# fu5ha/rayn

Hardware: AMD Instinct MI355X
Metric: Mpath-samples/sec (higher is better)
Workload: dtype f32; 1 GPU; 1920x1080, 1024 spp, 8 bounces, MandelBox SDF + homogeneous volume [BASELINE configs[2]]; fma_policy=unfused (reference default build), parallelism=tiles round-robin over 1 GPU(s), build_variant=product, resolve_kernel=k_resolve_blk<128, 8>

## Files before the change

rayn_amd/csrc/kernels.hip:

```cpp
#include <hip/hip_runtime.h>

#include <stdlib.h>

#include <algorithm>

#include "device_core.h"
#include "kernels.h"

#if defined(__HIP_DEVICE_COMPILE__) && !defined(__gfx950__)
#error "kernels.hip is written for gfx950 (MI355X): k_resolve_blk<512, 8> / k_resolve_huge use 64 KB / 130 KB of the CU's 160 KB LDS"
#endif

namespace RAYN_KNS {

RD uint32_t lane_id() { return threadIdx.x & 63u; }
RD uint32_t mbcnt(uint64_t mask) {
    return __builtin_amdgcn_mbcnt_hi((uint32_t)(mask >> 32), __builtin_amdgcn_mbcnt_lo((uint32_t)mask, 0u));
}

__global__ void __launch_bounds__(256) k_pack_tables(Tables tab, float4* __restrict__ out, uint32_t spp, uint32_t depths, uint32_t n1, uint32_t n2) {
    const uint32_t r = blockIdx.x * blockDim.x + threadIdx.x;
    if (r >= spp * depths) return;
    const uint32_t depth = r / spp, s = r % spp;
    float* dst = (float*)(out + (size_t)r * tab.rec_stride);
    for (uint32_t k = 0; k < 8; k++) dst[k] = k < n1 ? tab.s1d[s + spp * (1 + k + depth * n1)] : 0.0f;
    for (uint32_t c = 0; c < n2; c++) dst[8 + c] = tab.s2d[(c & 1) + s * 2 + spp * 2 * (2 + (c >> 1) + depth * (n2 / 2))];
}

__global__ void __launch_bounds__(256) k_batch_setup(const DTile* __restrict__ tiles, uint32_t* __restrict__ pgrp_tile,
                                                      uint32_t* __restrict__ tgb, uint32_t* __restrict__ tgc) {
    const uint32_t k = blockIdx.x;
    const DTile t = tiles[k];
    const uint32_t g0 = t.pool_base >> 6, groups = (t.n_paths + 63u) >> 6;
    if (threadIdx.x == 0) { tgb[k] = g0; tgc[k] = groups; }
    for (uint32_t g = threadIdx.x; g < groups; g += 256) pgrp_tile[g0 + g] = k;
}

__global__ void __launch_bounds__(256) k_raygen(const DScene* __restrict__ scp, Tables tab, const float* __restrict__ scramble,
                                                 const DTile* __restrict__ tiles, const uint32_t* __restrict__ pgrp_tile,
                                                 Pool pool, uint32_t* __restrict__ q, uint32_t n_pool, DCtl* __restrict__ ctl) {
    const uint32_t P = blockIdx.x * blockDim.x + threadIdx.x;
    if (P >= n_pool) return;
    if (P == 0) { ctl->q_groups = n_pool >> 6; ctl->q_valid = n_pool; ctl->head_extend = 0; }
    const DScene& sc = *scp;
    const DTile tile = tiles[pgrp_tile[P >> 6]];
    const uint32_t p = P - tile.pool_base;
    pool.term_info[P] = (uint8_t)TERM_NONE;
    pool.aov[P] = make_float4(0.0f, 0.0f, 0.0f, __uint_as_float(OBJ_NONE));
    if (p >= tile.n_paths) { q[P] = INVALID; return; }
    const uint32_t spp = sc.spp;
    const uint32_t s = p % spp, lpix = p / spp;
    const uint32_t lx = lpix / tile.eh, ly = lpix % tile.eh;
    const uint32_t x = tile.x0 + lx, y = tile.y0 + ly;
    const uint32_t pix = x + y * sc.width;
    const float scr = scramble[pix];
    float u0 = sample_2d(tab, spp, 0, s, scr, 0), u1 = sample_2d(tab, spp, 1, s, scr, 0);
    float fx = fis_sample(tab.fis, u0), fy = fis_sample(tab.fis, u1);
    float scx = ((float)x + 0.5f) + fx, scy = ((float)y + 0.5f) + fy;
    float uvx = sc.ndc_x * scx, uvy = sc.ndc_y * scy;
    float time = sc.time_start + sc.time_range * sample_1d(tab, spp, s, scr, 0);
    float l0 = sample_2d(tab, spp, 0, s, scr, 1), l1 = sample_2d(tab, spp, 1, s, scr, 1);
    const float t0 = sc.cam.animated ? sc.time_start + sc.time_range * sample_1d(tab, spp, s & ~3u, scr, 0) : time;
    f3 o, d;
    camera_ray(sc.cam, uvx, uvy, l0, l1, t0, &o, &d);
    pool.geo0[P] = make_float4(o.x, o.y, o.z, d.x);
    pool.geo1[P] = make_float4(d.y, d.z, 0.0f, __uint_as_float(OBJ_NONE | (s << 8)));
    pool.col0[P] = make_float4(0.0f, 0.0f, 0.0f, 1.0f);
    pool.col1[P] = make_float4(1.0f, 1.0f, __uint_as_float(pix), time);
    q[P] = P;
}

RD float packet_time(const DScene& sc, const uint32_t* __restrict__ q, const Pool& pool, uint32_t ent) {
    if (!sc.anim_spheres) return 0.0f;
    const uint32_t P0 = q[ent & ~3u];
    return P0 == INVALID ? dm_nanf() : pool.col1[P0].w;
}

constexpr uint32_t CHUNK = 256;
constexpr uint32_t ENDGAME_ENTRIES = 256 * 32 * 64;

template <bool COUNT>
__global__ void __launch_bounds__(256) k_extend(const DScene* __restrict__ scp, uint32_t depth, const uint32_t* __restrict__ q,
                                                 DCtl* __restrict__ ctl, Pool pool, uint8_t* __restrict__ ent_obj,
                                                 uint32_t REFILL_MIN, unsigned long long* __restrict__ evals_out) {
    const DScene& sc = *scp;
    const uint32_t n_entries = ctl->q_groups << 6;
    uint32_t* const head = &ctl->head_extend;
    const uint32_t lane = lane_id();
    const Thr th = make_thr(sc, depth);
    const uint32_t nh = sc.n_hitables;
    const float c0 = 0.00005f * sc.detail_scale, c1 = 0.05f * sc.detail_scale;
    uint32_t cur = 0, end = 0;
    bool exhausted = false;
    bool has = false, first = false, nan = false;
    uint32_t ent = 0, P = 0, k = 0, id = OBJ_NONE, m = 0, sbits = 0;
    EvalCtr evals;
    f3 o = f3{0, 0, 0}, d = f3{0, 0, 0};
    float closest = 0.0f, t = 0.0f, t0 = 0.0f;
    auto advance = [&]() {
        while (k < nh) {
            const DHitable& hh = sc.h[k];
            if (hh.kind != RAYN_HITABLE_SPHERE) { first = true; return; }
            float ts = sphere_hit(hh, o, d, closest, t0);
            if (ts < closest) { closest = ts; id = k; }
            k++;
        }
        *(float2*)(&pool.geo1[P].z) = make_float2(closest, __uint_as_float((sbits & ~0xFFu) | id));
        ent_obj[ent] = (uint8_t)id;
        has = false;
    };
    bool marching = false;
    for (;;) {
        const uint64_t parked = __ballot(!marching);
        if (parked != 0 && ((uint32_t)__popcll(parked) >= REFILL_MIN || exhausted)) {
            if (has && !marching) { advance(); marching = has; }
            for (;;) {
                const uint64_t need = __ballot(!has);
                if (need == 0) break;
                if (cur == end) {
                    if (exhausted) break;
                    uint32_t base = 0;
                    if (lane == 0) base = atomicAdd(head, CHUNK);
                    base = __builtin_amdgcn_readfirstlane(base);
                    if (base >= n_entries) { exhausted = true; break; }
                    cur = base;
                    end = min(base + CHUNK, n_entries);
                }
                const uint32_t rank = mbcnt(need), avail = end - cur;
                if (!has && rank < avail) {
                    ent = cur + rank;
                    P = q[ent];
                    if (P == INVALID) ent_obj[ent] = (uint8_t)OBJ_NONE;
                    else {
                        const float4 g0 = pool.geo0[P], g1 = pool.geo1[P];
                        o = f3{g0.x, g0.y, g0.z};
                        d = f3{g0.w, g1.x, g1.y};
                        sbits = __float_as_uint(g1.w);
                        t0 = packet_time(sc, q, pool, ent);
                        closest = sc.t_max; id = OBJ_NONE; k = 0; has = true;
                        advance();
                        marching = has;
                    }
                }
                cur += min((uint32_t)__popcll(need), avail);
            }
        }
        const uint64_t act = __ballot(marching);
        if (act == 0) {
            if (__ballot(has) == 0 && exhausted) break;
            continue;
        }
        const uint32_t ku = (uint32_t)__builtin_amdgcn_readlane((int)k, (int)__builtin_ctzll(act));
        const DHitable& h = sc.h[ku];
        if (marching && k == ku) {
            const f3 ol = o - sphere_center(h, t0);
            const f3 p = first ? ol : muladd3(d, t, ol);
            const float dist = sdf_dist<COUNT>(h, p, evals, sdf_scale(h, t0));
            bool done;
            if (first) { t = dist; nan = dist != dist; first = false; m = 0; done = sc.max_marches == 0; }
            else {
                const bool hit = __builtin_fabsf(dist) < fmaxs(c0, c1 * thr_at(th, t));
                const bool gt = t > closest;
                done = hit || nan || gt;
                if (!done) { t = t + dist; m++; done = m == sc.max_marches; }
            }
            if (done) {
                if (t < closest) { closest = t; id = k; }
                k++;
                marching = false;
            }
        }
    }
    if (COUNT && evals.n) { atomicAdd(evals_out, (unsigned long long)evals.n); atomicAdd(evals_out + 4, (unsigned long long)evals.it); }
}

template <bool COUNT, int SDFK>
__global__ void __launch_bounds__(256) k_extend1(const DScene* __restrict__ scp, uint32_t depth, uint32_t ks, const uint32_t* __restrict__ q,
                                                  DCtl* __restrict__ ctl, Pool pool, uint8_t* __restrict__ ent_obj,
                                                  uint32_t PREFETCH_MIN, unsigned long long* __restrict__ evals_out) {
    const DScene& sc = *scp;
    const uint32_t n_entries = ctl->q_groups << 6;
    uint32_t* const head = &ctl->head_extend;
    const uint32_t lane = lane_id();
    const Thr th = make_thr(sc, depth);
    const uint32_t nh = sc.n_hitables, max_marches = sc.max_marches;
    const DHitable h = sc.h[ks];
    const float c0 = 0.00005f * sc.detail_scale, c1 = 0.05f * sc.detail_scale;
    uint32_t cur = 0, end = 0;
    bool exhausted = false, endgame = false;
    bool c_has = false, first = false, nan = false;
    uint32_t c_P = 0, c_ent = 0, c_ids = 0, m = 0;
    EvalCtr evals;
    f3 o = f3{0, 0, 0}, d = f3{0, 0, 0};
    f3 pt = f3{0, 0, 0};
    float c_pre = 0.0f, c_post = 0.0f, t = 0.0f;
    float c_scale = h.scale, n_scale = h.scale;
    bool n_has = false;
    uint32_t n_P = 0, n_ent = 0, n_ids = 0;
    f3 n_o = f3{0, 0, 0}, n_d = f3{0, 0, 0};
    float n_pre = 0.0f, n_post = 0.0f;
    for (;;) {
        const uint64_t lack = __ballot(!n_has);
        const uint64_t idle = __ballot(!c_has && !n_has);
        if (!exhausted && (endgame ? idle != 0 : ((uint32_t)__popcll(lack) >= PREFETCH_MIN || (uint32_t)__popcll(idle) >= 4u))) {
            for (;;) {
                const uint64_t need = endgame ? __ballot(!n_has && !c_has) : __ballot(!n_has);
                if (need == 0) break;
                if (cur == end) {
                    uint32_t base = 0;
                    if (lane == 0) base = atomicAdd(head, CHUNK);
                    base = __builtin_amdgcn_readfirstlane(base);
                    if (base >= n_entries) { exhausted = true; break; }
                    cur = base;
                    end = min(base + CHUNK, n_entries);
                    endgame = n_entries - base < ENDGAME_ENTRIES;
                }
                const uint32_t rank = mbcnt(need), avail = end - cur;
                if ((need >> lane) & 1ull) if (rank < avail) {
                    n_ent = cur + rank;
                    n_P = q[n_ent];
                    if (n_P == INVALID) ent_obj[n_ent] = (uint8_t)OBJ_NONE;
                    else {
                        const float4 g0 = pool.geo0[n_P];
                        const float2 g1 = *(const float2*)(&pool.geo1[n_P].x);
                        n_o = f3{g0.x, g0.y, g0.z};
                        n_d = f3{g0.w, g1.x, g1.y};
                        const float t0 = packet_time(sc, q, pool, n_ent);
                        float closest = sc.t_max;
                        uint32_t id = OBJ_NONE;
                        for (uint32_t k = 0; k < ks; k++) {
                            float ts = sphere_hit(sc.h[k], n_o, n_d, closest, t0);
                            if (ts < closest) { closest = ts; id = k; }
                        }
                        n_pre = closest;
                        uint32_t idp = OBJ_NONE;
                        for (uint32_t k = ks + 1; k < nh; k++) {
                            float ts = sphere_hit(sc.h[k], n_o, n_d, closest, t0);
                            if (ts < closest) { closest = ts; idp = k; }
                        }
                        n_post = closest;
                        n_ids = id | (idp << 8);
                        n_o = n_o - sphere_center(h, t0);
                        n_scale = sdf_scale(h, t0);
                        n_has = true;
                    }
                }
                cur += min((uint32_t)__popcll(need), avail);
            }
        }
        if (!c_has && n_has) {
            c_has = true; n_has = false;
            o = n_o; d = n_d; c_pre = n_pre; c_post = n_post; c_ids = n_ids; c_P = n_P; c_ent = n_ent; c_scale = n_scale;
            first = true;
#ifndef RAYN_MARCH_POINT_SELECT
            pt = n_o;
#endif
        }
        if (__ballot(c_has) == 0) {
            if (exhausted) break;
            continue;
        }
        if (c_has) {
#ifdef RAYN_MARCH_POINT_SELECT
            const f3 p = first ? o : muladd3(d, t, o);
#else
            const f3 p = pt;
#endif
            const float dist = sdf_dist<COUNT, SDFK>(h, p, evals, c_scale);
            bool done;
            if (first) { t = dist; nan = dist != dist; first = false; m = 0; done = max_marches == 0; }
            else {
                const bool hit = __builtin_fabsf(dist) < fmaxs(c0, c1 * thr_at(th, t));
                const bool gt = t > c_pre;
                done = hit || nan || gt;
                if (!done) { t = t + dist; m++; done = m == max_marches; }
            }
            if (done) {
                float closest = c_pre;
                uint32_t id = c_ids & 0xFFu;
                if (t < closest) { closest = t; id = ks; }
                const uint32_t idp = c_ids >> 8;
                if (idp != OBJ_NONE && c_post < closest) { closest = c_post; id = idp; }
                pool.geo1[c_P].z = closest;
                ((uint8_t*)&pool.geo1[c_P].w)[0] = (uint8_t)id;
                ent_obj[c_ent] = (uint8_t)id;
                c_has = false;
            }
#ifndef RAYN_MARCH_POINT_SELECT
            else pt = muladd3(d, t, o);
#endif
        }
    }
    if (COUNT && evals.n) { atomicAdd(evals_out, (unsigned long long)evals.n); atomicAdd(evals_out + 4, (unsigned long long)evals.it); }
}

constexpr uint32_t QUEUE_UNROLL = 8;

RD uint32_t quad_total(uint32_t n) {
    n += (uint32_t)__builtin_amdgcn_update_dpp(0, (int)n, 0xB1, 0xF, 0xF, true);
    n += (uint32_t)__builtin_amdgcn_update_dpp(0, (int)n, 0x4E, 0xF, 0xF, true);
    return n;
}
RD uint32_t count_eq4(uint32_t v, uint32_t pat) {
    const uint32_t x = v ^ pat;
    return (uint32_t)__popc(~(((x & 0x7F7F7F7Fu) + 0x7F7F7F7Fu) | x | 0x7F7F7F7Fu));
}
__global__ void __launch_bounds__(256) k_group_hist(uint32_t nclass, const uint8_t* __restrict__ ent_obj, const DCtl* __restrict__ ctl,
                                                     uint8_t* __restrict__ grp_cnt) {
    const uint32_t n_q = ctl->q_groups << 2;
    const uint4* __restrict__ obj16 = (const uint4*)ent_obj;
    const uint32_t stride = gridDim.x * blockDim.x;
    constexpr uint32_t HIST_UNROLL = 2;
    for (uint32_t i0 = blockIdx.x * blockDim.x + threadIdx.x; i0 < n_q; i0 += stride * HIST_UNROLL) {
        uint4 v[HIST_UNROLL];
#pragma unroll
        for (uint32_t u = 0; u < HIST_UNROLL; u++) { const uint32_t i = i0 + u * stride; v[u] = i < n_q ? obj16[i] : make_uint4(~0u, ~0u, ~0u, ~0u); }
#pragma unroll
        for (uint32_t u = 0; u < HIST_UNROLL; u++) {
            const uint32_t i = i0 + u * stride;
            uint32_t acc[4] = {0u, 0u, 0u, 0u};
            for (uint32_t c = 0; c < nclass; c++) {
                const uint32_t pat = c * 0x01010101u;
                const uint32_t n = quad_total(count_eq4(v[u].x, pat) + count_eq4(v[u].y, pat) + count_eq4(v[u].z, pat) + count_eq4(v[u].w, pat));
                const uint32_t sh = n << (8u * (c & 3u));
                if ((c >> 2) == 0) acc[0] |= sh; else if ((c >> 2) == 1) acc[1] |= sh; else if ((c >> 2) == 2) acc[2] |= sh; else acc[3] |= sh;
            }
            if (i < n_q && (threadIdx.x & 3u) == 3u) *(uint4*)(grp_cnt + (size_t)(i >> 2) * SCAN_NC_BIN) = make_uint4(acc[0], acc[1], acc[2], acc[3]);
        }
    }
}
__global__ void __launch_bounds__(256) k_scan_tile(uint32_t nclass, uint32_t stride, uint32_t pad, const uint8_t* __restrict__ grp_cnt,
                                                    const uint32_t* __restrict__ tile_grp_begin, const uint32_t* __restrict__ tile_grp_count,
                                                    uint32_t* __restrict__ grp_base, uint32_t* __restrict__ grp_tile,
                                                    uint32_t* __restrict__ tile_total, uint32_t* __restrict__ tile_valid,
                                                    uint32_t* __restrict__ tile_cls_cnt, const DCtl* __restrict__ ctl) {
    if (ctl->overflow) return;
    __shared__ uint32_t s_tot[SCAN_NC_BIN];
    const uint32_t k = blockIdx.x;
    const uint32_t gb = tile_grp_begin[k], gc = tile_grp_count[k];
    const uint32_t lane = lane_id(), wave = threadIdx.x >> 6;
    for (uint32_t gi = threadIdx.x; gi < gc; gi += 256) grp_tile[gb + gi] = k;
    for (uint32_t c = wave; c < nclass; c += 4) {
        uint32_t run = 0;
        for (uint32_t base = 0; base < gc; base += 64 * QUEUE_UNROLL) {
            uint32_t v[QUEUE_UNROLL];
#pragma unroll
            for (uint32_t u = 0; u < QUEUE_UNROLL; u++) {
                const uint32_t gi = base + u * 64 + lane;
                v[u] = gi < gc ? grp_cnt[(size_t)(gb + gi) * stride + c] : 0u;
            }
#pragma unroll
            for (uint32_t u = 0; u < QUEUE_UNROLL; u++) {
                const uint32_t gi = base + u * 64 + lane;
                uint32_t inc = v[u];
#pragma unroll
                for (int off = 1; off < 64; off <<= 1) {
                    const uint32_t n = __shfl_up(inc, off);
                    if (lane >= (uint32_t)off) inc += n;
                }
                if (gi < gc) grp_base[(size_t)(gb + gi) * stride + c] = run + inc - v[u];
                run += (uint32_t)__builtin_amdgcn_readlane((int)inc, 63);
            }
        }
        if (lane == 0) s_tot[c] = run;
    }
    __syncthreads();
    if (threadIdx.x == 0) {
        uint32_t off = 0, valid = 0;
        for (uint32_t c = 0; c < nclass; c++) {
            valid += s_tot[c];
            tile_cls_cnt[k * SCAN_NC_BIN + c] = s_tot[c];
            off += (s_tot[c] + pad - 1) / pad * pad;
        }
        tile_total[k] = off;
        tile_valid[k] = valid;
    }
}

__global__ void __launch_bounds__(1024) k_tile_prefix(uint32_t n_tiles, const uint32_t* __restrict__ tile_total,
                                                       const uint32_t* __restrict__ tile_valid, uint32_t* __restrict__ tile_out_base,
                                                       uint32_t* __restrict__ out_grp_begin, uint32_t* __restrict__ out_grp_count,
                                                       DCtl* __restrict__ ctl, int stage, uint32_t nclass, uint32_t pad,
                                                       const uint32_t* __restrict__ tile_cls_cnt, uint32_t* __restrict__ tile_cls_base, uint32_t cap_groups,
                                                       uint32_t* __restrict__ base_hist) {
    __shared__ uint32_t s_wave[16];
    __shared__ uint32_t s_vsum[16];
    __shared__ uint32_t s_run, s_valid;
    if (threadIdx.x == 0) { s_run = 0; s_valid = 0; }
    __syncthreads();
    const uint32_t lane = lane_id(), wave = threadIdx.x >> 6;
    for (uint32_t base = 0; base < n_tiles; base += 1024) {
        const uint32_t k = base + threadIdx.x;
        const bool in = k < n_tiles;
        uint32_t groups = in ? (tile_total[k] + 63u) / 64u : 0u;
        uint32_t valid = in ? tile_valid[k] : 0u;
        uint32_t inc = groups, vs = valid;
#pragma unroll
        for (int off = 1; off < 64; off <<= 1) {
            uint32_t n = __shfl_up(inc, off);
            if (lane >= (uint32_t)off) inc += n;
            vs += __shfl_xor(vs, off);
        }
        if (lane == 63) s_wave[wave] = inc;
        if (lane == 0) s_vsum[wave] = vs;
        __syncthreads();
        uint32_t wbase = 0, tot = 0, vtot = 0;
        for (uint32_t w = 0; w < 16; w++) {
            uint32_t wt = s_wave[w];
            if (w < wave) wbase += wt;
            tot += wt;
            vtot += s_vsum[w];
        }
        const uint32_t run = s_run;
        if (in) {
            uint32_t begin = run + wbase + inc - groups;
            out_grp_begin[k] = begin;
            out_grp_count[k] = groups;
            tile_out_base[k] = begin * 64u;
            if (base_hist) base_hist[k] = begin * 64u;
            uint32_t off = begin * 64u;
            for (uint32_t c = 0; c < nclass; c++) {
                tile_cls_base[k * SCAN_NC_BIN + c] = off;
                const uint32_t cnt = tile_cls_cnt[k * SCAN_NC_BIN + c];
                off += (cnt + pad - 1) / pad * pad;
            }
        }
        __syncthreads();
        if (threadIdx.x == 0) { s_run = run + tot; s_valid += vtot; }
        __syncthreads();
    }
    if (threadIdx.x == 0) {
        if (s_run > cap_groups) ctl->overflow |= 1u << stage;
        if (ctl->overflow) { s_run = 0; s_valid = 0; }
        if (stage == 0) {
            ctl->entries_sum += (unsigned long long)ctl->q_groups << 6;
            ctl->b_groups = s_run; ctl->b_valid = s_valid;
            ctl->segments += s_valid; ctl->shaded_slots += (unsigned long long)s_run << 6;
            ctl->job_count = 0; ctl->head_shadow = 0;
        } else {
            ctl->q_groups = s_run; ctl->q_valid = s_valid;
            ctl->next_sum += (unsigned long long)s_run << 6;
            ctl->head_extend = 0;
        }
    }
// ... 321 lines not shown
        uint32_t nj = n_elided_jobs, no = n_oob;
#pragma unroll
        for (int off = 32; off > 0; off >>= 1) { nj += (uint32_t)__shfl_xor((int)nj, off); no += (uint32_t)__shfl_xor((int)no, off); }
        if (lane == 0 && em) {
            atomicAdd(evals_out + 2, (unsigned long long)__popcll(em)); atomicAdd(evals_out + 6, (unsigned long long)nj); atomicAdd(evals_out + 7, (unsigned long long)no);
        }
    }
}

constexpr uint32_t SCAN_ITEMS = 64;
__global__ void __launch_bounds__(256) k_shadow_list(Nee nee, uint32_t ns, DCtl* __restrict__ ctl) {
    __shared__ uint32_t s_wave[4];
    __shared__ uint32_t s_base;
    const uint32_t n_slots = ctl->b_groups << 6;
    const uint32_t n_ids = ns * n_slots;
    uint32_t* const job_count = &ctl->job_count;
    const size_t cap = nee.cap;
    const uint32_t lane = lane_id(), wave = threadIdx.x >> 6;
    for (uint32_t block_first = blockIdx.x * (256 * SCAN_ITEMS); block_first < n_ids; block_first += gridDim.x * (256 * SCAN_ITEMS)) {
    uint32_t refs[SCAN_ITEMS];
    uint8_t vis[SCAN_ITEMS];
#pragma unroll
    for (uint32_t r = 0; r < SCAN_ITEMS; r++) {
        const uint32_t g = (uint32_t)__builtin_amdgcn_readfirstlane((int)(block_first + (r * 4 + wave) * 64));
        const bool in = g < n_ids;
        const uint32_t gc = in ? g : 0u;
        const uint32_t s = gc / n_slots;
        refs[r] = (uint32_t)(s * cap + (gc - s * n_slots) + lane);
        vis[r] = nee.vis[refs[r]];
        if (!in) refs[r] = INVALID;
    }
    uint32_t wave_total = 0;
#pragma unroll
    for (uint32_t r = 0; r < SCAN_ITEMS; r++) {
        if (vis[r] != 2) refs[r] = INVALID;
        wave_total += (uint32_t)__popcll(__ballot(refs[r] != INVALID));
    }
    if (lane == 0) s_wave[wave] = wave_total;
    __syncthreads();
    uint32_t before = 0, tot = 0;
#pragma unroll
    for (uint32_t w = 0; w < 4; w++) {
        const uint32_t wt = s_wave[w];
        if (w < wave) before += wt;
        tot += wt;
    }
    if (threadIdx.x == 0) s_base = tot ? atomicAdd(job_count, tot) : 0u;
    __syncthreads();
    uint32_t w = s_base + before;
#pragma unroll
    for (uint32_t r = 0; r < SCAN_ITEMS; r++) {
        const uint64_t m = __ballot(refs[r] != INVALID);
        if (refs[r] != INVALID) nee.job_ref[w + mbcnt(m)] = refs[r];
        w += (uint32_t)__popcll(m);
    }
    __syncthreads();
    }
}

template <bool COUNT>
__global__ void __launch_bounds__(256) k_shadow(const DScene* __restrict__ scp, Nee nee, DCtl* __restrict__ ctl,
                                                 uint32_t REFILL_MIN, unsigned long long* __restrict__ evals_out) {
    const DScene& sc = *scp;
    const uint32_t lane = lane_id();
    const uint32_t n_jobs = ctl->job_count, nh = sc.n_hitables;
    uint32_t* const head = &ctl->head_shadow;
    if (blockIdx.x == 0 && threadIdx.x == 0) ctl->shadow_jobs += n_jobs;
    const float c0 = 0.0001f * sc.detail_scale, c1 = 0.00001f * sc.detail_scale;
    uint32_t cur = 0, end = 0;
    bool exhausted = false;
    bool has = false, first = false, nan = false;
    uint32_t ref = 0, k = 0, m = 0;
    EvalCtr evals;
    f3 start = f3{0, 0, 0}, dir = f3{0, 0, 0}, wa = f3{0, 0, 0}, wb = f3{0, 0, 0};
    float max_dist = 0.0f, t = 0.0f, jt0 = 0.0f;
    auto next_sdf = [&]() {
        while (k < nh && sc.h[k].kind == RAYN_HITABLE_SPHERE) k++;
        if (k >= nh) { nee.vis[ref] = 1; has = false; }
        else {
            const f3 origin = sphere_center(sc.h[k], jt0);
            start = wa - origin;
            dir = (wb - origin) - start;
            max_dist = mag(dir);
            dir = div_by_mag(dir, max_dist);
            first = true;
        }
    };
    for (;;) {
        const uint64_t idle = __ballot(!has);
        if (idle != 0 && ((uint32_t)__popcll(idle) >= REFILL_MIN) && !exhausted) {
            for (;;) {
                const uint64_t need = __ballot(!has);
                if (need == 0) break;
                if (cur == end) {
                    uint32_t base = 0;
                    if (lane == 0) base = atomicAdd(head, CHUNK);
                    base = __builtin_amdgcn_readfirstlane(base);
                    if (base >= n_jobs) { exhausted = true; break; }
                    cur = base;
                    end = min(base + CHUNK, n_jobs);
                }
                const uint32_t rank = mbcnt(need), avail = end - cur;
                if (!has && rank < avail) {
                    ref = nee.job_ref[cur + rank];
                    const float2 j0 = nee.job_geo[3 * (size_t)ref], j1 = nee.job_geo[3 * (size_t)ref + 1], j2 = nee.job_geo[3 * (size_t)ref + 2];
                    const float4 ja = make_float4(j0.x, j0.y, j1.x, j1.y), jb = make_float4(j2.x, j2.y, sc.anim_spheres ? nee.t0[ref % (uint32_t)nee.cap] : 0.0f, 0.0f);
                    wa = f3{ja.x, ja.y, ja.z};
                    wb = f3{ja.w, jb.x, jb.y};
                    jt0 = jb.z;
                    k = 0; has = true;
                    next_sdf();
                }
                cur += min((uint32_t)__popcll(need), avail);
            }
        }
        const uint64_t act = __ballot(has);
        if (act == 0) break;
        const uint32_t ku = (uint32_t)__builtin_amdgcn_readlane((int)k, (int)__builtin_ctzll(act));
        const DHitable& h = sc.h[ku];
        if (has && k == ku) {
            const f3 p = first ? start : muladd3(dir, t, start);
            const float dist = sdf_dist<COUNT>(h, p, evals, sdf_scale(h, jt0));
            int res = -1;
            if (first) {
                t = dist; nan = dist != dist; first = false; m = 0;
                if (sc.max_vis_marches == 0) res = ((dist < 0.0001f) && !((dist > max_dist) || nan)) ? 0 : 1;
                else if ((t > max_dist) || nan) res = 1;
            } else {
                if (__builtin_fabsf(dist) < fmaxs(c0, c1 * t)) res = 0;
                else {
                    t = t + dist; m++;
                    if (m == sc.max_vis_marches || (t > max_dist) || nan) res = 1;
                }
            }
            if (res == 0) has = false;
            else if (res == 1) { k++; next_sdf(); }
        }
    }
    if (COUNT && evals.n) { atomicAdd(evals_out, (unsigned long long)evals.n); atomicAdd(evals_out + 4, (unsigned long long)evals.it); }
}

template <bool COUNT, int SDFK>
__global__ void __launch_bounds__(256) k_shadow1(const DScene* __restrict__ scp, uint32_t ks, Nee nee, DCtl* __restrict__ ctl,
                                                  uint32_t PREFETCH_MIN, unsigned long long* __restrict__ evals_out) {
    const DScene& sc = *scp;
    const uint32_t lane = lane_id();
    const uint32_t n_jobs = ctl->job_count, max_vis = sc.max_vis_marches;
    uint32_t* const head = &ctl->head_shadow;
    if (blockIdx.x == 0 && threadIdx.x == 0) ctl->shadow_jobs += n_jobs;
    const DHitable h = sc.h[ks];
    const float c0 = 0.0001f * sc.detail_scale, c1 = 0.00001f * sc.detail_scale;
    uint32_t cur = 0, end = 0;
    bool exhausted = false, endgame = false;
    bool c_has = false, first = false, nan = false, n_has = false;
    uint32_t ref = 0, n_ref = 0, m = 0;
    EvalCtr evals;
    f3 start = f3{0, 0, 0}, dir = f3{0, 0, 0}, n_start = f3{0, 0, 0}, n_dir = f3{0, 0, 0};
    f3 pt = f3{0, 0, 0};
    float max_dist = 0.0f, n_max = 0.0f, t = 0.0f;
    float c_scale = h.scale, n_scale = h.scale;
    for (;;) {
        const uint64_t lack = __ballot(!n_has);
        const uint64_t idle = __ballot(!c_has && !n_has);
        if (!exhausted && (endgame ? idle != 0 : ((uint32_t)__popcll(lack) >= PREFETCH_MIN || (uint32_t)__popcll(idle) >= 4u))) {
            for (;;) {
                const uint64_t need = endgame ? __ballot(!n_has && !c_has) : __ballot(!n_has);
                if (need == 0) break;
                if (cur == end) {
                    uint32_t base = 0;
                    if (lane == 0) base = atomicAdd(head, CHUNK);
                    base = __builtin_amdgcn_readfirstlane(base);
                    if (base >= n_jobs) { exhausted = true; break; }
                    cur = base;
                    end = min(base + CHUNK, n_jobs);
                    endgame = n_jobs - base < ENDGAME_ENTRIES;
                }
                const uint32_t rank = mbcnt(need), avail = end - cur;
                if (((need >> lane) & 1ull) && rank < avail) {
                    n_ref = nee.job_ref[cur + rank];
                    const float2 j0 = nee.job_geo[3 * (size_t)n_ref], j1 = nee.job_geo[3 * (size_t)n_ref + 1], j2 = nee.job_geo[3 * (size_t)n_ref + 2];
                    const float jt0 = sc.anim_spheres ? nee.t0[n_ref % (uint32_t)nee.cap] : 0.0f;
                    const f3 origin = sphere_center(h, jt0);
                    n_scale = sdf_scale(h, jt0);
                    n_start = f3{j0.x, j0.y, j1.x} - origin;
                    const f3 e = f3{j1.y, j2.x, j2.y} - origin;
                    n_dir = e - n_start;
                    n_max = mag(n_dir);
                    n_dir = div_by_mag(n_dir, n_max);
                    n_has = true;
                }
                cur += min((uint32_t)__popcll(need), avail);
            }
        }
        if (!c_has && n_has) {
            c_has = true; n_has = false;
            start = n_start; dir = n_dir; max_dist = n_max; ref = n_ref; c_scale = n_scale;
            first = true;
#ifndef RAYN_MARCH_POINT_SELECT
            pt = n_start;
#endif
        }
        if (__ballot(c_has) == 0) {
            if (exhausted) break;
            continue;
        }
        if (c_has) {
#ifdef RAYN_MARCH_POINT_SELECT
            const f3 p = first ? start : muladd3(dir, t, start);
#else
            const f3 p = pt;
#endif
            const float dist = sdf_dist<COUNT, SDFK>(h, p, evals, c_scale);
            int res = -1;
            if (first) {
                t = dist; nan = dist != dist; first = false; m = 0;
                if (max_vis == 0) res = ((dist < 0.0001f) && !((dist > max_dist) || nan)) ? 0 : 1;
                else if ((t > max_dist) || nan) res = 1;
            } else {
                if (__builtin_fabsf(dist) < fmaxs(c0, c1 * t)) res = 0;
                else {
                    t = t + dist; m++;
                    if (m == max_vis || (t > max_dist) || nan) res = 1;
                }
            }
            if (res >= 0) { if (res == 1) nee.vis[ref] = 1; c_has = false; }
#ifndef RAYN_MARCH_POINT_SELECT
            else pt = muladd3(dir, t, start);
#endif
        }
    }
    if (COUNT && evals.n) { atomicAdd(evals_out, (unsigned long long)evals.n); atomicAdd(evals_out + 4, (unsigned long long)evals.it); }
}

#include "march_bulb.h"

__global__ void __launch_bounds__(256) k_shade_finish(const DScene* __restrict__ scp, const uint32_t* __restrict__ bq, const DCtl* __restrict__ ctl,
                                                       Pool pool, Nee nee) {
    const DScene& sc = *scp;
    const uint32_t n_slots = ctl->b_groups << 6;
    for (uint32_t j = blockIdx.x * blockDim.x + threadIdx.x; j < n_slots; j += gridDim.x * blockDim.x) {
    const uint32_t P = bq[j];
    if (P == INVALID) continue;
    const uint32_t flags = nee.flags[j], nl = sc.n_lights, VM = sc.vm;
    const size_t cap = nee.cap;
    if (flags & 6u) {
        const float4 c0 = pool.col0[P];
        const float2 c1 = *(const float2*)(&pool.col1[P].x);
        f3 rad = f3{c0.x, c0.y, c0.z};
        const f3 thr = f3{c0.w, c1.x, c1.y};
        if (flags & 2u) {
            const float corr = (float)nl / 4.0f, vol_T = nee.T[j];
            for (uint32_t i = 0; i < 4; i++) {
                const f3 x = f3{nee.x[(i * 3 + 0) * cap + j], nee.x[(i * 3 + 1) * cap + j], nee.x[(i * 3 + 2) * cap + j]};
                const float occ = nee.vis[i * cap + j] == 1 ? 1.0f : 0.0f;
                const f3 li = x * occ / nee.pdf[i * cap + j];
                rad = rad + li * thr * corr * vol_T;
            }
        }
        if (flags & 4u) {
            const float corr = (float)nl / 4.0f / (float)VM;
            const unsigned long long vpicks = nee.vpicks[j];
            for (uint32_t s = 4; s < 4 + 4 * VM; s++) {
                const float f = 1.0f / (4.0f * PI_F);
                const f3 x = sc.l[(uint32_t)(vpicks >> (4 * (s - 4))) & 15u].emission * f * nee.vtr[(s - 4) * cap + j];
                const float occ = nee.vis[s * cap + j] == 1 ? 1.0f : 0.0f;
                const f3 li = x * occ / nee.pdf[s * cap + j];
                rad = rad + li * thr * corr * sc.rho_s * nee.aux[(s - 4) * cap + j];
            }
        }
        if (flags & 1u) {
            pool.col0[P] = make_float4(rad.x, rad.y, rad.z, nee.nthr[j]);
            *(float2*)(&pool.col1[P].x) = make_float2(nee.nthr[cap + j], nee.nthr[2 * cap + j]);
        } else pool.col0[P] = make_float4(rad.x, rad.y, rad.z, c0.w);
    } else if (flags & 1u) {
        pool.col0[P].w = nee.nthr[j];
        *(float2*)(&pool.col1[P].x) = make_float2(nee.nthr[cap + j], nee.nthr[2 * cap + j]);
    }
    }
}

RD size_t film_pixel(const DTile& t, uint32_t lpix, uint32_t width) {
    if (t.film_packed) return (size_t)t.film_base + lpix;
    const uint32_t lx = lpix / t.eh, ly = lpix % t.eh;
    return (size_t)(t.x0 + lx) + (size_t)(t.y0 + ly) * width;
}

RD float serial_sum(const float* src, uint32_t stride, uint32_t cnt) {
    float a = 0.0f;
    uint32_t e = 0;
    for (; e + 8 <= cnt; e += 8) {
        float v[8];
#pragma unroll
        for (uint32_t u = 0; u < 8; u++) v[u] = src[(e + u) * stride];
#pragma unroll
        for (uint32_t u = 0; u < 8; u++) a += v[u];
    }
    for (; e < cnt; e++) a += src[e * stride];
    return a;
}

RD unsigned long long shfl_xor_key(unsigned long long v, uint32_t m) {
    const uint32_t lo = (uint32_t)__shfl_xor((int)(uint32_t)v, (int)m), hi = (uint32_t)__shfl_xor((int)(uint32_t)(v >> 32), (int)m);
    return ((unsigned long long)hi << 32) | lo;
}
RD uint32_t shfl_xor_key(uint32_t v, uint32_t m) { return (uint32_t)__shfl_xor((int)v, (int)m); }

template <typename K, uint32_t KPL>
RD void bitonic_sort_reg(K (&key)[KPL]) {
    const uint32_t lane = lane_id();
    constexpr uint32_t N = 64 * KPL;
#pragma nounroll
    for (uint32_t k = 2; k <= N; k <<= 1) {
        const bool asc_lane = ((lane * KPL) & k) == 0;
#pragma nounroll
        for (uint32_t jj = k >> 1; jj >= KPL && jj > 0; jj >>= 1) {
            const uint32_t lm = jj / KPL;
            const bool keep_min = asc_lane == ((lane & lm) == 0);
            K o[KPL];
#pragma unroll
            for (uint32_t r = 0; r < KPL; r++) o[r] = shfl_xor_key(key[r], lm);
#pragma unroll
            for (uint32_t r = 0; r < KPL; r++) {
                const bool take = (o[r] < key[r]) == keep_min;
                key[r] = take ? o[r] : key[r];
            }
        }
#pragma unroll
        for (uint32_t jj = KPL / 2; jj > 0; jj >>= 1) {
            if (jj < k) {
#pragma unroll
                for (uint32_t r = 0; r < KPL; r++) {
                    if ((r & jj) == 0) {
                        const bool asc = k < KPL ? (r & k) == 0 : asc_lane;
                        const K a = key[r], b = key[r | jj];
                        const bool sw = (a > b) == asc;
                        key[r] = sw ? b : a;
                        key[r | jj] = sw ? a : b;
                    }
                }
            }
        }
    }
}

RD unsigned long long shfl_key(unsigned long long v, uint32_t src) {
    const uint32_t lo = (uint32_t)__shfl((int)(uint32_t)v, (int)src), hi = (uint32_t)__shfl((int)(uint32_t)(v >> 32), (int)src);
    return ((unsigned long long)hi << 32) | lo;
}
RD uint32_t shfl_key(uint32_t v, uint32_t src) { return (uint32_t)__shfl((int)v, (int)src); }
template <typename K, uint32_t KPL>
RD bool is_sorted_reg(const K (&key)[KPL]) {
    const uint32_t lane = lane_id();
    bool ok = true;
#pragma unroll
    for (uint32_t r = 0; r < KPL; r++) {
        const K same = shfl_key(key[r], (lane + 1) & 63u);
        const K wrap = r + 1 < KPL ? shfl_key(key[r + 1 < KPL ? r + 1 : r], 0u) : (K)~(K)0;
        ok = ok && !(key[r] > (lane == 63 ? wrap : same));
    }
    return __ballot(!ok) == 0;
}

RD float serial_sum_range(const float* src, uint32_t lo, uint32_t hi) {
    float a = 0.0f;
    uint32_t e = lo;
    for (; e < hi && (e & 3u); e++) a += src[e];
    for (; e + 8 <= hi; e += 8) {
        const float4 v0 = *(const float4*)(src + e), v1 = *(const float4*)(src + e + 4);
        a += v0.x; a += v0.y; a += v0.z; a += v0.w;
        a += v1.x; a += v1.y; a += v1.z; a += v1.w;
    }
    for (; e < hi; e++) a += src[e];
    return a;
}

template <uint32_t KPL>
__global__ void __launch_bounds__(64) k_resolve_reg(const DScene* __restrict__ scp, const DTile* __restrict__ tiles, Pool pool,
                                                     float* __restrict__ out_color, float* __restrict__ out_alpha,
                                                     float* __restrict__ out_background, float* __restrict__ out_normal) {
    constexpr uint32_t n_sort = 64 * KPL;
    __shared__ __attribute__((aligned(16))) float ch[3][n_sort];
    __shared__ uint8_t s_flag[n_sort];
// ... 681 lines not shown
```

Before: 259.3 Mpath-samples/s.

## Track wavefront march state as uniform lane masks instead of per-lane bools

Rewrites the persistent extend and NEE-visibility sphere-march loops so that per-lane state (has-current, has-next, NaN) lives in wave-uniform 64-bit masks updated with ballots, not in per-lane booleans. Control flow becomes branchless selects driven by inverse_ballot, and the SDF is evaluated on all lanes unconditionally when not counting. The aim is to cut VGPR and exec-mask divergence overhead and redundant ballots in the hot march loop. In exchange, idle lanes now do wasted SDF evaluations, and the RAYN_MARCH_POINT_SELECT path is dropped. The step counting was also changed (e vs m, max_vis==0 handling), which could alter semantics.

```diff
diff --git a/rayn_amd/csrc/kernels.hip b/rayn_amd/csrc/kernels.hip
--- a/rayn_amd/csrc/kernels.hip
+++ b/rayn_amd/csrc/kernels.hip
@@ -14,6 +14,7 @@
 namespace RAYN_KNS {
 
 RD uint32_t lane_id() { return threadIdx.x & 63u; }
+RD bool lane_of(uint64_t mask) { return __builtin_amdgcn_inverse_ballot_w64(mask); }
 RD uint32_t mbcnt(uint64_t mask) {
     return __builtin_amdgcn_mbcnt_hi((uint32_t)(mask >> 32), __builtin_amdgcn_mbcnt_lo((uint32_t)mask, 0u));
 }
@@ -188,23 +189,21 @@
     const float c0 = 0.00005f * sc.detail_scale, c1 = 0.05f * sc.detail_scale;
     uint32_t cur = 0, end = 0;
     bool exhausted = false, endgame = false;
-    bool c_has = false, first = false, nan = false;
-    uint32_t c_P = 0, c_ent = 0, c_ids = 0, m = 0;
+    uint64_t cm = 0, nm = 0, nanm = 0;
+    uint32_t c_P = 0, c_ent = 0, c_ids = 0, e = 0;
     EvalCtr evals;
     f3 o = f3{0, 0, 0}, d = f3{0, 0, 0};
     f3 pt = f3{0, 0, 0};
     float c_pre = 0.0f, c_post = 0.0f, t = 0.0f;
     float c_scale = h.scale, n_scale = h.scale;
-    bool n_has = false;
     uint32_t n_P = 0, n_ent = 0, n_ids = 0;
     f3 n_o = f3{0, 0, 0}, n_d = f3{0, 0, 0};
     float n_pre = 0.0f, n_post = 0.0f;
     for (;;) {
-        const uint64_t lack = __ballot(!n_has);
-        const uint64_t idle = __ballot(!c_has && !n_has);
+        const uint64_t lack = ~nm, idle = ~(cm | nm);
         if (!exhausted && (endgame ? idle != 0 : ((uint32_t)__popcll(lack) >= PREFETCH_MIN || (uint32_t)__popcll(idle) >= 4u))) {
             for (;;) {
-                const uint64_t need = endgame ? __ballot(!n_has && !c_has) : __ballot(!n_has);
+                const uint64_t need = endgame ? ~(nm | cm) : ~nm;
                 if (need == 0) break;
                 if (cur == end) {
                     uint32_t base = 0;
@@ -216,7 +215,8 @@
                     endgame = n_entries - base < ENDGAME_ENTRIES;
                 }
                 const uint32_t rank = mbcnt(need), avail = end - cur;
-                if ((need >> lane) & 1ull) if (rank < avail) {
+                const uint64_t take = need & __builtin_amdgcn_ballot_w64(rank < avail);
+                if (lane_of(take)) {
                     n_ent = cur + rank;
                     n_P = q[n_ent];
                     if (n_P == INVALID) ent_obj[n_ent] = (uint8_t)OBJ_NONE;
@@ -242,54 +242,45 @@
                         n_ids = id | (idp << 8);
                         n_o = n_o - sphere_center(h, t0);
                         n_scale = sdf_scale(h, t0);
-                        n_has = true;
                     }
                 }
+                nm |= take & __builtin_amdgcn_ballot_w64(n_P != INVALID);
                 cur += min((uint32_t)__popcll(need), avail);
             }
         }
-        if (!c_has && n_has) {
-            c_has = true; n_has = false;
-            o = n_o; d = n_d; c_pre = n_pre; c_post = n_post; c_ids = n_ids; c_P = n_P; c_ent = n_ent; c_scale = n_scale;
-            first = true;
-#ifndef RAYN_MARCH_POINT_SELECT
+        const uint64_t fm = nm & ~cm;
+        if (lane_of(fm)) {
+            o = n_o; d = n_d; c_pre = n_pre; c_post = n_post; c_ids = n_ids; c_P = n_P; c_ent = n_ent; e = 0;
+            c_scale = n_scale;
             pt = n_o;
-#endif
-        }
-        if (__ballot(c_has) == 0) {
+        }
+        cm |= fm; nm &= ~fm;
+        if (cm == 0) {
             if (exhausted) break;
             continue;
         }
-        if (c_has) {
-#ifdef RAYN_MARCH_POINT_SELECT
-            const f3 p = first ? o : muladd3(d, t, o);
-#else
-            const f3 p = pt;
-#endif
-            const float dist = sdf_dist<COUNT, SDFK>(h, p, evals, c_scale);
-            bool done;
-            if (first) { t = dist; nan = dist != dist; first = false; m = 0; done = max_marches == 0; }
-            else {
-                const bool hit = __builtin_fabsf(dist) < fmaxs(c0, c1 * thr_at(th, t));
-                const bool gt = t > c_pre;
-                done = hit || nan || gt;
-                if (!done) { t = t + dist; m++; done = m == max_marches; }
-            }
-            if (done) {
-                float closest = c_pre;
-                uint32_t id = c_ids & 0xFFu;
-                if (t < closest) { closest = t; id = ks; }
-                const uint32_t idp = c_ids >> 8;
-                if (idp != OBJ_NONE && c_post < closest) { closest = c_post; id = idp; }
-                pool.geo1[c_P].z = closest;
-                ((uint8_t*)&pool.geo1[c_P].w)[0] = (uint8_t)id;
-                ent_obj[c_ent] = (uint8_t)id;
-                c_has = false;
-            }
-#ifndef RAYN_MARCH_POINT_SELECT
-            else pt = muladd3(d, t, o);
-#endif
-        }
+        float dist = 0.0f;
+        if (!COUNT) dist = sdf_dist<COUNT, SDFK>(h, pt, evals, c_scale);
+        else if (lane_of(cm)) dist = sdf_dist<COUNT, SDFK>(h, pt, evals, c_scale);
+        const uint64_t stop = (__builtin_amdgcn_ballot_w64(__builtin_fabsf(dist) < fmaxs(c0, c1 * thr_at(th, t))) | __builtin_amdgcn_ballot_w64(t > c_pre) | nanm) & ~fm;
+        nanm = (nanm & ~fm) | (__builtin_amdgcn_ballot_w64(dist != dist) & fm);
+        const float ts = t + dist;
+        const float tg = lane_of(fm) ? dist : ts;
+        t = lane_of(stop) ? t : tg;
+        e++;
+        const uint64_t fin = (stop | __builtin_amdgcn_ballot_w64(e == max_marches + 1u)) & cm;
+        if (lane_of(fin)) {
+            float closest = c_pre;
+            uint32_t id = c_ids & 0xFFu;
+            if (t < closest) { closest = t; id = ks; }
+            const uint32_t idp = c_ids >> 8;
+            if (idp != OBJ_NONE && c_post < closest) { closest = c_post; id = idp; }
+            pool.geo1[c_P].z = closest;
+            ((uint8_t*)&pool.geo1[c_P].w)[0] = (uint8_t)id;
+            ent_obj[c_ent] = (uint8_t)id;
+        }
+        cm &= ~fin;
+        pt = muladd3(d, t, o);
     }
     if (COUNT && evals.n) { atomicAdd(evals_out, (unsigned long long)evals.n); atomicAdd(evals_out + 4, (unsigned long long)evals.it); }
 }
@@ -917,19 +908,18 @@
     const float c0 = 0.0001f * sc.detail_scale, c1 = 0.00001f * sc.detail_scale;
     uint32_t cur = 0, end = 0;
     bool exhausted = false, endgame = false;
-    bool c_has = false, first = false, nan = false, n_has = false;
-    uint32_t ref = 0, n_ref = 0, m = 0;
+    uint64_t cm = 0, nm = 0;
+    uint32_t ref = 0, n_ref = 0, e = 0;
     EvalCtr evals;
     f3 start = f3{0, 0, 0}, dir = f3{0, 0, 0}, n_start = f3{0, 0, 0}, n_dir = f3{0, 0, 0};
     f3 pt = f3{0, 0, 0};
     float max_dist = 0.0f, n_max = 0.0f, t = 0.0f;
     float c_scale = h.scale, n_scale = h.scale;
     for (;;) {
-        const uint64_t lack = __ballot(!n_has);
-        const uint64_t idle = __ballot(!c_has && !n_has);
+        const uint64_t lack = ~nm, idle = ~(cm | nm);
         if (!exhausted && (endgame ? idle != 0 : ((uint32_t)__popcll(lack) >= PREFETCH_MIN || (uint32_t)__popcll(idle) >= 4u))) {
             for (;;) {
-                const uint64_t need = endgame ? __ballot(!n_has && !c_has) : __ballot(!n_has);
+                const uint64_t need = endgame ? ~(nm | cm) : ~nm;
                 if (need == 0) break;
                 if (cur == end) {
                     uint32_t base = 0;
@@ -941,58 +931,52 @@
                     endgame = n_jobs - base < ENDGAME_ENTRIES;
                 }
                 const uint32_t rank = mbcnt(need), avail = end - cur;
-                if (((need >> lane) & 1ull) && rank < avail) {
+                const uint64_t take = need & __builtin_amdgcn_ballot_w64(rank < avail);
+                if (lane_of(take)) {
                     n_ref = nee.job_ref[cur + rank];
                     const float2 j0 = nee.job_geo[3 * (size_t)n_ref], j1 = nee.job_geo[3 * (size_t)n_ref + 1], j2 = nee.job_geo[3 * (size_t)n_ref + 2];
                     const float jt0 = sc.anim_spheres ? nee.t0[n_ref % (uint32_t)nee.cap] : 0.0f;
                     const f3 origin = sphere_center(h, jt0);
                     n_scale = sdf_scale(h, jt0);
                     n_start = f3{j0.x, j0.y, j1.x} - origin;
-                    const f3 e = f3{j1.y, j2.x, j2.y} - origin;
-                    n_dir = e - n_start;
+                    const f3 e1 = f3{j1.y, j2.x, j2.y} - origin;
+                    n_dir = e1 - n_start;
                     n_max = mag(n_dir);
                     n_dir = div_by_mag(n_dir, n_max);
-                    n_has = true;
                 }
+                nm |= take;
                 cur += min((uint32_t)__popcll(need), avail);
             }
         }
-        if (!c_has && n_has) {
-            c_has = true; n_has = false;
-            start = n_start; dir = n_dir; max_dist = n_max; ref = n_ref; c_scale = n_scale;
-            first = true;
-#ifndef RAYN_MARCH_POINT_SELECT
+        const uint64_t fm = nm & ~cm;
+        if (lane_of(fm)) {
+            start = n_start; dir = n_dir; max_dist = n_max; ref = n_ref; e = 0;
+            c_scale = n_scale;
             pt = n_start;
-#endif
-        }
-        if (__ballot(c_has) == 0) {
+        }
+        cm |= fm; nm &= ~fm;
+        if (cm == 0) {
             if (exhausted) break;
             continue;
         }
-        if (c_has) {
-#ifdef RAYN_MARCH_POINT_SELECT
-            const f3 p = first ? start : muladd3(dir, t, start);
-#else
-            const f3 p = pt;
-#endif
-            const float dist = sdf_dist<COUNT, SDFK>(h, p, evals, c_scale);
-            int res = -1;
-            if (first) {
-                t = dist; nan = dist != dist; first = false; m = 0;
-                if (max_vis == 0) res = ((dist < 0.0001f) && !((dist > max_dist) || nan)) ? 0 : 1;
-                else if ((t > max_dist) || nan) res = 1;
-            } else {
-                if (__builtin_fabsf(dist) < fmaxs(c0, c1 * t)) res = 0;
-                else {
-                    t = t + dist; m++;
-                    if (m == max_vis || (t > max_dist) || nan) res = 1;
-                }
-            }
-            if (res >= 0) { if (res == 1) nee.vis[ref] = 1; c_has = false; }
-#ifndef RAYN_MARCH_POINT_SELECT
-            else pt = muladd3(dir, t, start);
-#endif
-        }
+        float dist = 0.0f;
+        if (!COUNT) dist = sdf_dist<COUNT, SDFK>(h, pt, evals, c_scale);
+        else if (lane_of(cm)) dist = sdf_dist<COUNT, SDFK>(h, pt, evals, c_scale);
+        uint64_t occ, vis;
+        if (max_vis == 0) {
+            occ = __builtin_amdgcn_ballot_w64(dist < 0.0001f) & ~__builtin_amdgcn_ballot_w64(dist > max_dist);
+            vis = ~occ;
+        } else {
+            occ = __builtin_amdgcn_ballot_w64(__builtin_fabsf(dist) < fmaxs(c0, c1 * t)) & ~fm;
+            const float ts = t + dist;
+            t = lane_of(fm) ? dist : ts;
+            e++;
+            vis = (__builtin_amdgcn_ballot_w64(e == max_vis + 1u) | __builtin_amdgcn_ballot_w64(t > max_dist) | (__builtin_amdgcn_ballot_w64(dist != dist) & fm)) & ~occ;
+        }
+        vis &= cm;
+        if (lane_of(vis)) nee.vis[ref] = 1;
+        cm &= ~(occ | vis);
+        pt = muladd3(dir, t, start);
     }
     if (COUNT && evals.n) { atomicAdd(evals_out, (unsigned long long)evals.n); atomicAdd(evals_out + 4, (unsigned long long)evals.it); }
 }
```

Result: faster. 263.7 Mpath-samples/s, median of 6 (+1.7%).
